# Nikhil-Kulkarni/RayTrace-miniapp

Measured on AMD Instinct MI355X. Metric: ray_steps_per_sec, higher is better.
Workload: dtype f32+f64

## Files before the change

### raytrace-miniapp_amd/csrc/rt_launch.hip

```cpp
#include "rt_path.hip"
#include "rt_freq.hip"
#include "rt_fused.hip"
#include "rt_spec.hip"
#include "rt_step.hip"
#include "rt_step_seeds.hip"
#include "rt_fused_step.hip"
#include "rt_step_scan.hip"
#include "rt_step_scan_seeds.hip"
#include "rt_step_ase_seeds.hip"

#include "rt_runtime.h"
#include "rt_run_shape.h"

#include <atomic>
#include <cstdlib>
#include <cstring>
#include <map>
#include <mutex>

using namespace rtr;

namespace {

int allow_lds(const void *kernel, int device, size_t bytes, size_t limit)
// ... 707 lines not shown
        out->pass_nslot      = s.nslot;
        out->pass_lds        = s.flds;
        out->pass_grid       = s.fgrid;
        out->pass_fetch_shift = s.fetch_shift;
        return RT_OK;
    }
    const PassKind kind   = pass_kind(f);
    const PassShape ps    = pass_shape(kind, f, t);
    out->pass_kind        = (int) kind;
    out->pass_wg_waves    = ps.wg_waves;
    out->pass_in_lds      = ps.in_lds;
    out->pass_nslot       = ps.nslot;
    out->pass_lds         = ps.lds;
    out->pass_grid        = ps.grid;
    out->pass_fetch_shift = ps.fetch_shift;
    return RT_OK;
}

#ifdef RT_WAVETIMES
int rt_hip_debug_wavetimes(unsigned long long *summary8, unsigned long long *end8192, unsigned long long *dry8192)
{
    HIP_TRY(hipDeviceSynchronize());
    HIP_TRY(hipMemcpyFromSymbol(summary8, HIP_SYMBOL(rt::g_wt), 8 * sizeof(unsigned long long)));
    HIP_TRY(hipMemcpyFromSymbol(end8192, HIP_SYMBOL(rt::g_wt_end), 8192 * sizeof(unsigned long long)));
    HIP_TRY(hipMemcpyFromSymbol(dry8192, HIP_SYMBOL(rt::g_wt_dry), 8192 * sizeof(unsigned long long)));
    unsigned long long init[8] = { ~0ull, 0, ~0ull, 0, ~0ull, 0, 0, 0 };
    HIP_TRY(hipMemcpyToSymbol(HIP_SYMBOL(rt::g_wt), init, sizeof(init)));
    return RT_OK;
}
int rt_hip_debug_wavetrace(unsigned long long *trace, int samples, unsigned *blocks)
{
    HIP_TRY(hipDeviceSynchronize());
    if (samples != rt::WT_TRACE)
        return fail_arg("rt_hip_debug_wavetrace: samples");
    if (blocks)
        HIP_TRY(hipMemcpyFromSymbol(blocks, HIP_SYMBOL(rt::g_wt_blocks), sizeof(unsigned) * 8192 * rt::WT_TRACE * 6));
    HIP_TRY(hipMemcpyFromSymbol(trace, HIP_SYMBOL(rt::g_wt_trace), sizeof(unsigned long long) * 8192 * rt::WT_TRACE));
    void *sym = nullptr;
    HIP_TRY(hipGetSymbolAddress(&sym, HIP_SYMBOL(rt::g_wt_trace)));
    HIP_TRY(hipMemset(sym, 0, sizeof(unsigned long long) * 8192 * rt::WT_TRACE));
    return RT_OK;
}
int rt_hip_debug_publish(unsigned long long *pub4, unsigned long long *vm)
{
    HIP_TRY(hipDeviceSynchronize());
    HIP_TRY(hipMemcpyFromSymbol(pub4, HIP_SYMBOL(rt::g_wt_pub), sizeof(unsigned long long) * 8192 * 4));
    HIP_TRY(hipMemcpyFromSymbol(vm, HIP_SYMBOL(rt::g_wt_vm), sizeof(unsigned long long) * 8192));
    void *sym = nullptr;
    HIP_TRY(hipGetSymbolAddress(&sym, HIP_SYMBOL(rt::g_wt_pub)));
    HIP_TRY(hipMemset(sym, 0, sizeof(unsigned long long) * 8192 * 4));
    HIP_TRY(hipGetSymbolAddress(&sym, HIP_SYMBOL(rt::g_wt_vm)));
    HIP_TRY(hipMemset(sym, 0, sizeof(unsigned long long) * 8192));
    return RT_OK;
}
int rt_hip_debug_freqtimes(unsigned long long *times, unsigned *n_waves)
{
    HIP_TRY(hipDeviceSynchronize());
    HIP_TRY(hipMemcpyFromSymbol(times, HIP_SYMBOL(rt::g_ft), 6 * 8192 * sizeof(unsigned long long)));
    HIP_TRY(hipMemcpyFromSymbol(n_waves, HIP_SYMBOL(rt::g_ft_n), sizeof(unsigned)));
    const unsigned zero = 0;
    HIP_TRY(hipMemcpyToSymbol(HIP_SYMBOL(rt::g_ft_n), &zero, sizeof(zero)));
    return RT_OK;
}
#endif

#ifdef RT_INSTRUMENT
int rt_hip_debug_ray_iters(unsigned short *out, unsigned long long n)
{
    HIP_TRY(hipDeviceSynchronize());
    HIP_TRY(hipMemcpyFromSymbol(out, HIP_SYMBOL(rt::g_ray_iters), (size_t) n * sizeof(unsigned short)));
    return RT_OK;
}
#endif
#ifdef RT_INSTRUMENT
int rt_hip_debug_prune_counters(unsigned long long *out4)
{
    HIP_TRY(hipDeviceSynchronize());
    HIP_TRY(hipMemcpyFromSymbol(out4, HIP_SYMBOL(rt::g_prune), 4 * sizeof(unsigned long long)));
    unsigned long long z[4] = { 0 };
    HIP_TRY(hipMemcpyToSymbol(HIP_SYMBOL(rt::g_prune), z, sizeof(z)));
    return RT_OK;
}
#endif
#if defined(RT_INSTRUMENT) || defined(RT_TIMEBLOCKS)
int rt_hip_debug_counters(unsigned long long *out8)
{
    HIP_TRY(hipDeviceSynchronize());
    HIP_TRY(hipMemcpyFromSymbol(out8, HIP_SYMBOL(rt::g_inst), 8 * sizeof(unsigned long long)));
    unsigned long long z[8] = { 0 };
    HIP_TRY(hipMemcpyToSymbol(HIP_SYMBOL(rt::g_inst), z, sizeof(z)));
    return RT_OK;
}
#endif

}
```

### raytrace-miniapp_amd/csrc/rt_march.hip

```cpp
#pragma once
#include "rt_math.h"

#include <cfloat>

namespace rt {

enum : int { ST_IDLE = 0, ST_CELL = 1, ST_XSETUP = 2, ST_STEP = 3, ST_DONE = 4 };

typedef double f64x2 __attribute__((ext_vector_type(2)));
typedef float f32x4 __attribute__((ext_vector_type(4)));
typedef unsigned u32x4 __attribute__((ext_vector_type(4)));

__device__ __forceinline__ unsigned div_magic(unsigned x, unsigned mul, unsigned sh)
{
    return mul ? __umulhi(x, mul) >> sh : x;
}
__device__ __forceinline__ void grid_index(const DevRays &R, unsigned ridx, unsigned &i, unsigned &j, unsigned &k,
                                           unsigned &m)
{
    const unsigned ijkm = (unsigned) (R.first + (long long) ridx * R.stride);
    const unsigned q1   = div_magic(ijkm, R.div_mul[0], R.div_sh[0]);
    m                   = ijkm - q1 * (unsigned) R.ngb;
    const unsigned q2   = div_magic(q1, R.div_mul[1], R.div_sh[1]);
    k                   = q1 - q2 * (unsigned) R.nga;
    i                   = div_magic(q2, R.div_mul[2], R.div_sh[2]);
    j                   = q2 - i * (unsigned) R.ngy;
}

__device__ __forceinline__ void load_ray(const DevRays &R, unsigned ridx, rt_ray &ray, float &ta, float &tb,
                                         bool want_tan)
{
    if (R.list) {
        ray = R.list[ridx];
        if (want_tan) {
            ta = R.sxy[2 * (size_t) ridx];
            tb = R.sxy[2 * (size_t) ridx + 1];
        }
    } else {
        unsigned i, j, k, m;
        grid_index(R, ridx, i, j, k, m);
        ray.x      = (float) R.gx[i];
        ray.y      = (float) R.gy[j];
        ray.a      = (float) R.ga[k];
        ray.b      = (float) R.gb[m];
        if (want_tan) {
            ta = R.tan_a[k];
            tb = R.tan_b[m];
        }
    }
}

__device__ __attribute__((noinline)) float tan_wide(float x)
{
    if (!(fabsf(x) <= FLT_MAX))
        return x - x;
    return (float) tan((double) x);
}
__device__ __attribute__((noinline)) float atan_wide(float x)
{
    const float A0 = 3.3333334327e-01f, A1 = -2.0000000298e-01f, A2 = 1.4285714924e-01f, A3 = -1.1111110449e-01f,
                A4 = 9.0908870101e-02f, A5 = -7.6918758452e-02f, A6 = 6.6610731184e-02f, A7 = -5.8335702866e-02f,
                A8 = 4.9768779427e-02f, A9 = -3.6531571299e-02f, A10 = 1.6285819933e-02f;
    const unsigned hx = __float_as_uint(x), ix = hx & 0x7fffffffu;
    const bool neg = (hx >> 31) != 0u;
    if (ix >= 0x4c000000u) {
        if (ix > 0x7f800000u)
            return x + x;
        const float r = 1.5707962513e+00f + 7.5497894159e-08f;
        return neg ? -r : r;
    }
    float hi, lo;
    x = fabsf(x);
    if (ix < 0x3f980000u) {
        if (ix < 0x3f300000u) {
            hi = 4.6364760399e-01f;
            lo = 5.0121582440e-09f;
            x  = (2.0f * x - 1.0f) / (2.0f + x);
        } else {
            hi = 7.8539812565e-01f;
            lo = 3.7748947079e-08f;
            x  = (x - 1.0f) / (x + 1.0f);
        }
    } else {
        if (ix < 0x401c0000u) {
            hi = 9.8279368877e-01f;
            lo = 3.4473217170e-08f;
            x  = (x - 1.5f) / (1.0f + 1.5f * x);
        } else {
            hi = 1.5707962513e+00f;
            lo = 7.5497894159e-08f;
// ... 165 lines not shown
    const unsigned long long nth = (unsigned long long) gridDim.x * blockDim.x;
    for (unsigned long long t = tid; t < (unsigned long long) n_fast + n_other; t += nth) {
        const unsigned u = t < n_fast ? lo + (unsigned) t : (unsigned) (t - n_fast) << 8;
        float q          = __uint_as_float(u);
        const float a    = inv_norm(q);
        asm volatile("" : "+v"(q));
        const float b = 1.0f / sqrtf(q);
        checked++;
        if (__float_as_uint(a) != __float_as_uint(b) && !(a != a && b != b))
            bad++;
    }
    for (unsigned long long t = tid; t < (4ull << 23); t += nth) {
        float n       = __uint_as_float(0x3e800000u + (unsigned) t);
        const float a = fdiv_one_nr(n);
        asm volatile("" : "+v"(n));
        const float b = 1.0f / n;
        checked++;
        bad += __float_as_uint(a) != __float_as_uint(b) ? 1 : 0;
    }
    for (unsigned long long t = tid; t < (1ull << 28); t += nth) {
        const unsigned h0 = selftest_hash((unsigned) t * 2u + 1u), h1 = selftest_hash((unsigned) t * 2u + 0x9e3779b9u);
        const int ea = -84 + (int) (h0 % 84u), eb = -78 + (int) (h1 % 122u);
        if (ea - eb >= 96 || eb - ea >= 96 || ea - eb < -120)
            continue;
        float x = __uint_as_float(((unsigned) (ea + 127) << 23) | (selftest_hash(h0) & 0x7fffffu));
        float y = __uint_as_float(((unsigned) (eb + 127) << 23) | (selftest_hash(h1) & 0x7fffffu));
        const float a = fdiv_nr(x, y);
        asm volatile("" : "+v"(x), "+v"(y));
        const float b = x / y;
        checked++;
        bad += __float_as_uint(a) != __float_as_uint(b) ? 1 : 0;
    }
    if (tid == 0) {
        float inf = __uint_as_float(0x7f800000u), qnan = __uint_as_float(0x7fc00000u), big = 3.0e38f;
        asm volatile("" : "+v"(inf), "+v"(qnan), "+v"(big));
        const unsigned pio2 = 0x3fc90fdbu;
        const float t0 = tanf_flt32_kernel(inf), t1 = tanf_flt32_kernel(-inf), t2 = tanf_flt32_kernel(qnan), t3 = tan_wide(inf),
                    t4 = tan_wide(qnan), t5 = tanf_flt32_kernel(big);
        const float a0 = atanf_flt32_kernel(inf), a1 = atanf_flt32_kernel(-inf), a2 = atanf_flt32_kernel(qnan),
                    a3 = atanf_flt32_kernel(big), a4 = atanf_flt32_kernel(-big);
        checked += 11;
        bad += (t0 == t0) + (t1 == t1) + (t2 == t2) + (t3 == t3) + (t4 == t4) + (__float_as_uint(t5) == 0x7fc12345u);
        bad += (__float_as_uint(a0) != pio2) + (__float_as_uint(a1) != (pio2 | 0x80000000u)) + (a2 == a2) +
               (__float_as_uint(a3) != pio2) + (__float_as_uint(a4) != (pio2 | 0x80000000u));
    }
    atomicAdd(&counts[0], checked);
    atomicAdd(&counts[1], bad);
}

extern "C" __global__ void __launch_bounds__(256) rt_tan_kernel(const rt_ray *rays, unsigned long long n, float *sxy)
{
    unsigned long long i = (unsigned long long) blockIdx.x * blockDim.x + threadIdx.x;
    if (i < n) {
        rt_ray r       = rays[i];
        sxy[2 * i]     = tanf_flt32_kernel(1e-3f * r.a);
        sxy[2 * i + 1] = tanf_flt32_kernel(1e-3f * r.b);
    }
}

__device__ __forceinline__ int bisect_interval(const Interval *iv, int n, double v)
{
    int lo = 0, hi = n - 1;
    while (hi - lo != 1) {
        int mid = (hi + lo) / 2;
        if (iv[mid].hi >= v)
            hi = mid;
        else
            lo = mid;
    }
    return hi;
}
__device__ __forceinline__ int guess_interval(int n, float g0, float inv_h, float v)
{
    return (int) fminf(fmaxf((v - g0) * inv_h, 0.0f), (float) (n - 2)) + 1;
}

#ifdef RT_INSTRUMENT
__device__ unsigned long long g_inst[8];
__device__ unsigned long long g_prune[4];
__device__ unsigned short g_ray_iters[1u << 23];
#endif
#ifdef RT_TIMEBLOCKS
__device__ unsigned long long g_inst[8];
#endif
#ifdef RT_WAVETIMES
__device__ unsigned long long g_wt[8];
__device__ unsigned long long g_wt_end[8192], g_wt_dry[8192];
constexpr int WT_TRACE = 64;
__device__ unsigned long long g_wt_trace[8192][WT_TRACE];
__device__ unsigned g_wt_blocks[8192][WT_TRACE][6];
__device__ unsigned long long g_wt_pub[8192][4];
__device__ unsigned long long g_wt_vm[8192];
#endif
#if defined(RT_INSTRUMENT) || defined(RT_TIMEBLOCKS) || defined(RT_WAVETIMES)
struct MarchDiag {
    static __device__ __forceinline__ unsigned wave_number() { return blockIdx.x * (blockDim.x >> 6) + (threadIdx.x >> 6); }
    static __device__ __forceinline__ bool first_active_lane()
    {
        return (int) (threadIdx.x & 63) == __ffsll((long long) __ballot(1)) - 1;
    }
#ifdef RT_INSTRUMENT
    unsigned w[3] = { 0, 0, 0 }, a[3] = { 0, 0, 0 }, ray_iters = 0;
#endif
#if defined(RT_TIMEBLOCKS) || defined(RT_WAVEBLOCKS)
    unsigned long long tb_acc[6] = { 0, 0, 0, 0, 0, 0 }, tb_last = __builtin_readcyclecounter(), tb_iters = 0;
#endif
#ifdef RT_WAVETIMES
    const unsigned long long wt_start = __builtin_amdgcn_s_memrealtime();
    unsigned long long wt_dry = 0, pub_t0 = 0;
    unsigned wt_a_runs = 0, wt_b_runs = 0, wave_iter = 0;
#endif
    __device__ __forceinline__ void tick(int i)
    {
#ifdef RT_INSTRUMENT
        a[i]++;
        w[i] += first_active_lane() ? 1u : 0u;
#endif
    }
    __device__ __forceinline__ void mark(int i)
    {
#if defined(RT_TIMEBLOCKS) || defined(RT_WAVEBLOCKS)
        const unsigned long long now = __builtin_readcyclecounter();
        tb_acc[i] += now - tb_last;
        tb_last = now;
#endif
    }
    __device__ __forceinline__ void iteration(int st, int lane, int n_idle)
    {
#ifdef RT_INSTRUMENT
        ray_iters += st != ST_IDLE ? 1u : 0u;
#endif
#ifdef RT_TIMEBLOCKS
        tb_iters++;
#endif
#ifdef RT_WAVETIMES
        if ((++wave_iter & 15u) == 0u) {
            const unsigned wid = wave_number(), smp = wave_iter >> 4;
            if (lane == 0 && wid < 8192u && smp < (unsigned) WT_TRACE) {
                g_wt_trace[wid][smp] = (__builtin_amdgcn_s_memrealtime() & 0xffffffffffull) | ((unsigned long long) (WAVE - n_idle) << 40) |
                                       ((unsigned long long) wt_a_runs << 48) | ((unsigned long long) wt_b_runs << 56);
                g_wt_trace[wid][0] = smp;
#ifdef RT_WAVEBLOCKS
                for (int b = 0; b < 6; b++)
                    g_wt_blocks[wid][smp][b] = (unsigned) tb_acc[b];
#endif
            }
#ifdef RT_WAVEBLOCKS
            for (int b = 0; b < 6; b++)
                tb_acc[b] = 0;
#endif
            wt_a_runs = wt_b_runs = 0;
        }
#endif
    }
    __device__ __forceinline__ void counters_dry()
    {
#ifdef RT_WAVETIMES
        wt_dry = __builtin_amdgcn_s_memrealtime();
#endif
    }
    __device__ __forceinline__ void blocks_run(bool a_runs, bool lane_wants_b)
    {
#ifdef RT_WAVETIMES
        wt_a_runs += a_runs ? 1u : 0u;
        wt_b_runs += __ballot(lane_wants_b) != 0ull ? 1u : 0u;
#endif
    }
    __device__ __forceinline__ void ray_retired(unsigned ridx)
    {
#ifdef RT_INSTRUMENT
        if (ridx < (1u << 23))
            g_ray_iters[ridx] = (unsigned short) (ray_iters < 65535u ? ray_iters : 65535u);
        ray_iters = 0;
#endif
    }
    __device__ __forceinline__ void publish_begin()
    {
#ifdef RT_WAVETIMES
        pub_t0 = __builtin_amdgcn_s_memrealtime();
#endif
    }
    __device__ __forceinline__ void publish_stores_landed()
    {
#ifdef RT_WAVETIMES
        const unsigned long long now = __builtin_amdgcn_s_memrealtime();
        atomicAdd(&g_wt_vm[wave_number() & 8191u], now - pub_t0);
        pub_t0 = now;
#endif
    }
    __device__ __forceinline__ void publish_end()
    {
#ifdef RT_WAVETIMES
        const unsigned long long dt = __builtin_amdgcn_s_memrealtime() - pub_t0;
        unsigned long long *q       = g_wt_pub[wave_number() & 8191u];
        atomicAdd(&q[0], dt);
        atomicAdd(&q[1], 1ull);
        atomicMax(&q[3], dt);
#endif
    }
    static __device__ __forceinline__ void push_retry()
    {
#ifdef RT_WAVETIMES
        atomicAdd(&g_wt_pub[wave_number() & 8191u][2], 1ull);
#endif
    }
    __device__ __forceinline__ void tiny_dividend()
    {
#ifdef RT_INSTRUMENT
        if (first_active_lane())
            atomicAdd(&g_inst[6], 1ull);
#endif
    }
    __device__ __forceinline__ void prune(int i)
    {
#ifdef RT_INSTRUMENT
        if (first_active_lane())
            atomicAdd(&g_prune[i], 1ull);
#endif
    }
    __device__ __forceinline__ void wave_end(int lane)
    {
#ifdef RT_WAVETIMES
        if (lane == 0) {
            const unsigned long long wt_end = __builtin_amdgcn_s_memrealtime();
            atomicMin(&g_wt[0], wt_start);
            atomicMax(&g_wt[1], wt_start);
            const unsigned n = atomicAdd((unsigned *) &g_wt[6], 1u);
            if (n < 8192)
                g_wt_end[n] = wt_end | ((unsigned long long) (threadIdx.x >> 6) << 56), g_wt_dry[n] = wt_dry;
        }
#endif
#ifdef RT_TIMEBLOCKS
        if (lane == 0) {
            for (int i = 0; i < 6; i++)
                atomicAdd(&g_inst[i], tb_acc[i]);
            atomicAdd(&g_inst[7], tb_iters);
        }
#endif
#ifdef RT_INSTRUMENT
        for (int i = 0; i < 3; i++) {
            const unsigned tw = wave_sum_u32(w[i]), ta = wave_sum_u32(a[i]);
            if (lane == 0) {
                atomicAdd(&g_inst[2 * i], (unsigned long long) tw);
                atomicAdd(&g_inst[2 * i + 1], (unsigned long long) ta);
            }
        }
#endif
    }
};
#else
struct MarchDiag {
    __device__ __forceinline__ void tick(int) {}
    __device__ __forceinline__ void mark(int) {}
    __device__ __forceinline__ void iteration(int, int, int) {}
    __device__ __forceinline__ void counters_dry() {}
    __device__ __forceinline__ void blocks_run(bool, bool) {}
    __device__ __forceinline__ void ray_retired(unsigned) {}
    __device__ __forceinline__ void publish_begin() {}
    __device__ __forceinline__ void publish_stores_landed() {}
    __device__ __forceinline__ void publish_end() {}
    static __device__ __forceinline__ void push_retry() {}
    __device__ __forceinline__ void tiny_dividend() {}
    __device__ __forceinline__ void prune(int) {}
    __device__ __forceinline__ void wave_end(int) {}
};
#endif

struct TileList {
    unsigned *head;
    unsigned *next;
    unsigned *lnode;
    unsigned *nalloc;
    unsigned cap;
    unsigned *rem;
    unsigned *marching;
    unsigned n_waves;
    unsigned split;
    unsigned k_part;
};
constexpr unsigned TILE_NONE = 0xffffffffu;
constexpr unsigned TILE_PART_FLAG = 1u << 30, TILE_PART_SHIFT = 28, TILE_ID_MASK = (1u << TILE_PART_SHIFT) - 1u;
__device__ __forceinline__ unsigned tile_node(unsigned entry)
{
    return (entry & TILE_ID_MASK) * 4u + ((entry & TILE_PART_FLAG) ? (entry >> TILE_PART_SHIFT) & 3u : 0u);
}
constexpr unsigned TILE_REF_GLOBAL = 1u << 31;
__device__ __forceinline__ void tile_push(const TileList &T, unsigned tile)
{
    const unsigned id = __hip_atomic_fetch_add(T.nalloc, 1u, __ATOMIC_RELAXED, __HIP_MEMORY_SCOPE_WORKGROUP);
    unsigned old      = __hip_atomic_load(T.head, __ATOMIC_RELAXED, __HIP_MEMORY_SCOPE_WORKGROUP);
    if (id < T.cap) {
        __hip_atomic_store(&T.lnode[2u * id], tile, __ATOMIC_RELAXED, __HIP_MEMORY_SCOPE_WORKGROUP);
        for (;;) {
            __hip_atomic_store(&T.lnode[2u * id + 1u], old, __ATOMIC_RELAXED, __HIP_MEMORY_SCOPE_WORKGROUP);
            asm volatile("s_waitcnt lgkmcnt(0)" ::: "memory");
            if (__hip_atomic_compare_exchange_strong(T.head, &old, id, __ATOMIC_RELAXED, __ATOMIC_RELAXED, __HIP_MEMORY_SCOPE_WORKGROUP))
                return;
            MarchDiag::push_retry();
        }
    }
    tile |= TILE_REF_GLOBAL;
    for (;;) {
        __hip_atomic_store(&T.next[tile_node(tile & ~TILE_REF_GLOBAL)], old, __ATOMIC_RELAXED, __HIP_MEMORY_SCOPE_WORKGROUP);
        asm volatile("s_waitcnt vmcnt(0)" ::: "memory");
        if (__hip_atomic_compare_exchange_strong(T.head, &old, tile, __ATOMIC_RELAXED, __ATOMIC_RELAXED, __HIP_MEMORY_SCOPE_WORKGROUP))
            return;
        MarchDiag::push_retry();
    }
}
__device__ __forceinline__ void tile_publish(const TileList &T, unsigned tile)
{
    bool parts = T.split == 2u;
    if (T.split == 1u)
        parts = __hip_atomic_load(T.head, __ATOMIC_RELAXED, __HIP_MEMORY_SCOPE_WORKGROUP) == TILE_NONE &&
                __hip_atomic_load(T.marching, __ATOMIC_RELAXED, __HIP_MEMORY_SCOPE_WORKGROUP) * 8u <= T.n_waves;
    if (parts && T.k_part != 0u) {
        for (unsigned q = 0; q < 4u; q++)
            tile_push(T, tile | (q << TILE_PART_SHIFT) | TILE_PART_FLAG);
    } else {
        tile_push(T, tile);
    }
}
__device__ __forceinline__ unsigned tile_pop(const TileList &T)
{
    unsigned old = __hip_atomic_load(T.head, __ATOMIC_RELAXED, __HIP_MEMORY_SCOPE_WORKGROUP);
    while (old != TILE_NONE) {
        const unsigned nxt = (old & TILE_REF_GLOBAL)
                                 ? __hip_atomic_load(&T.next[tile_node(old & ~TILE_REF_GLOBAL)], __ATOMIC_RELAXED, __HIP_MEMORY_SCOPE_WORKGROUP)
                                 : __hip_atomic_load(&T.lnode[2u * old + 1u], __ATOMIC_RELAXED, __HIP_MEMORY_SCOPE_WORKGROUP);
        if (__hip_atomic_compare_exchange_strong(T.head, &old, nxt, __ATOMIC_RELAXED, __ATOMIC_RELAXED, __HIP_MEMORY_SCOPE_WORKGROUP))
            break;
    }
    if (old == TILE_NONE)
        return TILE_NONE;
    return (old & TILE_REF_GLOBAL) ? (old & ~TILE_REF_GLOBAL) : __hip_atomic_load(&T.lnode[2u * old], __ATOMIC_RELAXED, __HIP_MEMORY_SCOPE_WORKGROUP);
}

template <bool LDS_TAB> __device__ __forceinline__ void march_load_tables(const DevParams &P, unsigned char *lds_raw)
{
    if (LDS_TAB) {
        const uint4 *src = reinterpret_cast<const uint4 *>(P.blob);
        uint4 *dst       = reinterpret_cast<uint4 *>(lds_raw);
        const unsigned n16 = P.blob_bytes / 16, step = blockDim.x;
        for (unsigned i0 = threadIdx.x; i0 < n16; i0 += 8 * step) {
            uint4 v[8];
#pragma unroll
            for (int u = 0; u < 8; u++) {
                const unsigned i = i0 + (unsigned) u * step;
                v[u]             = src[i < n16 ? i : i0];
            }
#pragma unroll
            for (int u = 0; u < 8; u++) {
                const unsigned i = i0 + (unsigned) u * step;
                if (i < n16)
                    dst[i] = v[u];
            }
        }
        __syncthreads();
    }
}

enum : int { MARCH_OPT_PRUNE = 1, MARCH_OPT_NO_NTEST = 2, MARCH_OPT_PRUNE_H24 = 4, MARCH_OPT_SCAN = 8 };
constexpr unsigned SCAN_BND_BYTES = 20u, SCAN_BND_ROW = WAVE * SCAN_BND_BYTES;
RT_HD inline size_t scan_bnd_off(unsigned ridx, int j, int L)
{
    return ((size_t) (ridx >> 6) * (size_t) (L - 1) + (size_t) (j - 1)) * SCAN_BND_ROW + (size_t) (ridx & 63u) * SCAN_BND_BYTES;
}
RT_HD inline size_t scan_bnd_bytes(unsigned long long n_rays, int L)
{
    return (size_t) ((n_rays + WAVE - 1) / WAVE) * (size_t) (L > 1 ? L - 1 : 0) * SCAN_BND_ROW;
}
template <bool LDS_TAB, bool BOUNDED, bool FUSED, int MODE = 0, int OPT = 0>
__device__ __forceinline__ void march_wave(const DevParams &P, unsigned char *lds_raw, const TileList done)
{
    const int lane        = lane_id();
    const int L           = P.L;
    const int S           = L * RT_N_SUB;
    const unsigned n_rays = P.ray_end;
    const bool backward   = MODE == 1 ? true : ((MODE == 2 || MODE == 3) ? false : P.method == 1);
    const bool use_emis   = MODE == 1 ? true : ((MODE == 2 || MODE == 4) ? false : P.use_emis != 0);
    const bool path_on    = MODE == 0 ? P.path_on != 0 : false;
    const unsigned CH     = P.chunk;
    constexpr int REFILL  = 8;

    const unsigned char *tab = LDS_TAB ? lds_raw : P.blob;
    const BlobGain *hdr = reinterpret_cast<const BlobGain *>(tab);
    const unsigned lds_base = LDS_TAB ? (unsigned) (size_t) (__attribute__((address_space(3))) unsigned char *) lds_raw : 0u;

    static_assert(RT_N_SUB == 3, "sub-segment ends are tabulated for three sub-segments");
    float zs0 = (P.dz0 * (0.0f + 1.0f) / RT_N_SUB), zs1 = (P.dz0 * (1.0f + 1.0f) / RT_N_SUB),
          zs2 = (P.dz0 * (2.0f + 1.0f) / RT_N_SUB);
    asm volatile("" : "+v"(zs0), "+v"(zs1), "+v"(zs2));

    unsigned chunk_next = 0, chunk_end = 0;
    unsigned fetched_end = 0, cur_slot = 0;
    unsigned cslot       = 0;
    bool more           = true;
    const unsigned n_launch_rays = n_rays - P.ray_begin;
    const unsigned n_chunks      = (n_launch_rays + CH - 1) / CH;
    unsigned shard = blockIdx.x & 7u, shards_seen_empty = 0;
    const unsigned n_main = n_chunks - (P.late_chunks < n_chunks ? P.late_chunks : 0u);
    const bool late_wave  = (unsigned) __builtin_amdgcn_readfirstlane((int) (threadIdx.x >> 6)) - P.late_first < P.late_waves;
    unsigned zone = 0;

    int st        = ST_IDLE;
    unsigned ridx = 0;
    int seg = 0, iz = 0, ii = 0;
    float z = 0.0f, z_stop = 0.0f;
    float px = 0, py = 0, pz = 0, sx = 0, sy = 0, sz = 1;
    float gacc = 0, eacc = 0;
    int cell_last = 0, sub = 0;
    unsigned char *recp = P.rec;
    unsigned lane12     = 0;
    BlobGain G    = hdr[1];
    unsigned steps = 0;
    bool escaped = false, mirror = false;
    unsigned any_bits = 0;
    int c00 = 0;
    float f00 = 1, f10 = 1, f01 = 1, f11 = 1;
    double dnx0 = 0, dnx1 = 0, dny0 = 0, dny1 = 0;
    f64x2 ix0 = { 0.0, 1.0 }, iy0 = { 0.0, 1.0 };
    f32x4 ix1 = { 1.0f, 0.0f, 0.0f, 0.0f }, iy1 = { 1.0f, 0.0f, 0.0f, 0.0f };
    float g0 = 0, E0 = 0;
    float dzrem = 0, zc = 0, path = 0;
    float rx = 0, ry = 0, rz = 0, n = 0, n0 = 0, gxn = 0, gyn = 0, lim2 = 0, dzcap = 0, hsum = 0;
    unsigned tot_steps = 0, tot_esc = 0, tot_rays = 0, tot_skip = 0;
    unsigned spin = 0;
    MarchDiag diag;
    for (;;) {
        diag.mark(5);
        unsigned long long idle2      = __ballot(st == ST_IDLE);
        const unsigned long long idle = idle2;
        const int n_idle              = (int) __popcll(idle);
        diag.iteration(st, lane, n_idle);
        if (!BOUNDED) {
            if (((++spin) & 0xfffu) == 0u && spin >= P.spin_limit) {
                spin = 0;
                if (st != ST_IDLE) {
                    escaped = true;
                    sx = sy = sz = 0.0f;
                    st           = ST_CELL;
                }
            }
        }
        if (more && (n_idle >= REFILL)) {
            const int rank = (int) __builtin_amdgcn_mbcnt_hi((unsigned) (idle >> 32),
                                                             __builtin_amdgcn_mbcnt_lo((unsigned) idle, 0u));
            int need = n_idle, off = 0;
            bool got = false;
            while (need > 0) {
                if (chunk_next == chunk_end && !(FUSED && chunk_next != fetched_end)) {
                    unsigned c = 0;
                    if (lane == 0)
                        c = atomicAdd(&P.ctl->next_tile[P.launch_id][shard][zone * 8u], 1u);
                    c = (unsigned) __builtin_amdgcn_readfirstlane((int) c) * 8u + shard + zone * n_main;
                    if (c >= (zone ? n_chunks : n_main)) {
                        if (++shards_seen_empty == 8) {
                            if (zone == 0u && late_wave && n_main < n_chunks) {
                                zone              = 1u;
                                shards_seen_empty = 0;
                                continue;
                            }
                            more = false;
                            diag.counters_dry();
                            break;
                        }
                        shard = (shard + 1) & 7u;
                        continue;
                    }
                    chunk_next = P.ray_begin + c * CH;
                    chunk_end  = (n_rays - chunk_next < CH) ? n_rays : chunk_next + CH;
                    if (FUSED) {
                        fetched_end = chunk_end;
                        chunk_end   = chunk_next;
                    }
                }
                if (FUSED && chunk_next == chunk_end) {
                    const unsigned in_use    = lane < 32 ? __hip_atomic_load(&done.rem[lane], __ATOMIC_RELAXED, __HIP_MEMORY_SCOPE_WAVEFRONT) : 1u;
                    const unsigned slot_busy = ~(unsigned) __ballot(lane < 32 && in_use == 0u);
                    const int fs = __builtin_ffs((int) ~slot_busy) - 1;
                    if (fs < 0)
                        break;
                    chunk_end = fetched_end - chunk_next < (unsigned) WAVE ? fetched_end : chunk_next + (unsigned) WAVE;
                    cur_slot  = (unsigned) fs;
                    if (lane == 0)
                        __hip_atomic_store(&done.rem[fs], chunk_end - chunk_next, __ATOMIC_RELAXED, __HIP_MEMORY_SCOPE_WAVEFRONT);
                }
                int avail = (int) (chunk_end - chunk_next);
                int take  = avail < need ? avail : need;
                if (st == ST_IDLE && !got && rank >= off && rank < off + take) {
                    ridx = chunk_next + (unsigned) (rank - off);
                    got  = true;
                    if (FUSED)
                        cslot = cur_slot;
                }
                chunk_next += (unsigned) take;
                need -= take;
                off += take;
            }
            if (!BOUNDED && __ballot(got) != 0ull)
                spin = 0;
            if (got) {
                rt_ray ray;
                float ta = 0, tb = 0;
                load_ray(P.rays, ridx, ray, ta, tb, true);
                px = ray.x;
                py = ray.y;
                pz = 0.0f;
                sx = ta;
                sy = tb;
                sz = 1.0f;
                if (backward) {
                    sx = -sx;
                    sy = -sy;
                    sz = -sz;
                }
                renormalise(sx, sy, sz);
                const BlobGain G0 = hdr[backward ? P.N - 1 : 1];
                const float dsum  = sx + sy + sz;
                const bool wild   = ((px != px) | (py != py) | (dsum != dsum)) &
                                  !((px < G0.lo_x) | (px > G0.hi_x) | (py < G0.lo_y) | (py > G0.hi_y));
                if (path_on) {
                    float *pp = P.path + (size_t) ridx * 3 * (size_t) (S + 1) + 3 * (size_t) (backward ? S : 0);
                    pp[0]     = px;
                    pp[1]     = py;
                }
                recp      = P.rec + rec_slot_off(ridx, backward ? S - 1 : 0, P.rec_stride);
                lane12    = (ridx & 63u) * 12u;
                seg       = 0;
                iz        = 0;
                ii        = backward ? P.N - 1 : 1;
                G         = G0;
                z         = 0.0f;
                z_stop    = zs0;
                gacc      = 0.0f;
                eacc      = 0.0f;
                cell_last = 0;
                steps     = 0;
                escaped   = wild;
                sx        = wild ? 0.0f : sx;
                sy        = wild ? 0.0f : sy;
                sz        = wild ? 0.0f : sz;
                any_bits  = P.no_skip;
                sub       = 0;
                st        = ST_CELL;
            }
            idle2 = __ballot(st == ST_IDLE);
        }
        if (idle2 == ~0ull) {
            if (!more)
                break;
        } else {

        diag.mark(0);
        const unsigned long long want_a = __ballot(st == ST_CELL);
        int park_at = (int) P.park;
        if (!more || (int) P.park > 12 || REFILL > 8) {
            const int n_live = WAVE - (int) __popcll(idle2);
            const int fifth  = (n_live * 13 + 63) >> 6;
            park_at          = fifth < (int) P.park ? fifth : (int) P.park;
        }
        const bool do_a = (int) __popcll(want_a) >= park_at || (~(idle2 | want_a)) == 0ull;
        diag.blocks_run(do_a && want_a != 0ull, st == ST_XSETUP);
        if (do_a && st == ST_CELL) {
            bool in_seg        = !escaped & (z < 0.995f * z_stop);
            if (!in_seg) {
#ifndef RT_ABL_NOSTORE
                *reinterpret_cast<RecSlot *>(recp) = RecSlot{ gacc, eacc, cell_last };
#endif
                recp += backward ? -(int) REC_SLOT_ROW : (int) REC_SLOT_ROW;
                any_bits |= (__float_as_uint(gacc) | __float_as_uint(eacc)) & 0x7fffffffu;
                if (path_on) {
                    float *pp = P.path + (size_t) ridx * 3 * (size_t) (S + 1);
                    for (int zz = iz; zz < (escaped ? RT_N_SUB : iz + 1); zz++) {
                        const int idx = RT_N_SUB * (ii - 1) + (backward ? RT_N_SUB - zz - 1 : zz + 1);
                        pp[3 * idx]     = px;
                        pp[3 * idx + 1] = py;
                    }
                }
                gacc      = 0.0f;
                eacc      = 0.0f;
                cell_last = 0;
                sub++;
                const bool wrap = iz == RT_N_SUB - 1;
                const bool fin  = escaped | (sub == S);
                iz              = wrap ? 0 : iz + 1;
                z               = wrap ? 0.0f : z;
                st              = fin ? ST_DONE : ST_CELL;
                if (wrap & !fin) {
                    if (OPT & MARCH_OPT_SCAN) {
                        unsigned char *bnd = reinterpret_cast<unsigned char *>(((unsigned long long) P.pad_march[1] << 32) | (unsigned long long) P.pad_march[0]);
                        float *q           = reinterpret_cast<float *>(bnd + scan_bnd_off(ridx, seg + 1, L));
                        q[0]               = px;
                        q[1]               = py;
                        q[2]               = sx;
                        q[3]               = sy;
                        q[4]               = sz;
                    }
                    seg++;
                    ii = backward ? P.N - seg - 1 : seg + 1;
                    G  = hdr[ii];
                }
                z_stop = iz == 0 ? zs0 : (iz == 1 ? zs1 : zs2);
                in_seg = !fin & (z < 0.995f * z_stop);
            }
            diag.mark(1);
            if ((st == ST_CELL) & in_seg) {
                if ((px < G.lo_x) | (px > G.hi_x) | (py < G.lo_y) | (py > G.hi_y) | (sz * sz <= 0.01f)) {
                    escaped = true;
                } else {
                    mirror              = G.mirror_y != 0;
                    const Interval *ivx = reinterpret_cast<const Interval *>(tab + G.off_ix);
                    const Interval *ivy = reinterpret_cast<const Interval *>(tab + G.off_iy);
                    f64x2 tx, ty;
                    u32x4 q00, q10, q01, q11;
                    auto gather = [&](int k1, int k2, int c) {
                        const unsigned ox = (unsigned) G.off_ix + (unsigned) k1 * (unsigned) sizeof(Interval);
                        const unsigned oy = (unsigned) G.off_iy + (unsigned) k2 * (unsigned) sizeof(Interval);
                        const unsigned oa = (unsigned) G.off_node + (unsigned) c * (unsigned) sizeof(Node);
                        const unsigned ob = oa + (unsigned) G.Nx * (unsigned) sizeof(Node);
                        if (LDS_TAB) {
                            asm volatile("ds_read_b128 %0, %10\n\t"
                                         "ds_read_b128 %1, %10 offset:16\n\t"
                                         "ds_read_b128 %2, %10 offset:32\n\t"
                                         "ds_read_b128 %3, %11\n\t"
                                         "ds_read_b128 %4, %11 offset:16\n\t"
                                         "ds_read_b128 %5, %11 offset:32\n\t"
                                         "ds_read_b128 %6, %12\n\t"
                                         "ds_read_b128 %7, %12 offset:16\n\t"
                                         "ds_read_b128 %8, %13\n\t"
                                         "ds_read_b128 %9, %13 offset:16\n\t"
                                         "s_waitcnt lgkmcnt(0)"
                                         : "=&v"(ix0), "=&v"(ix1), "=&v"(tx), "=&v"(iy0), "=&v"(iy1), "=&v"(ty), "=&v"(q00), "=&v"(q10),
                                           "=&v"(q01), "=&v"(q11)
                                         : "v"(lds_base + ox), "v"(lds_base + oy), "v"(lds_base + oa), "v"(lds_base + ob));
                        } else {
                            const unsigned char *t = tab;
                            ix0 = *reinterpret_cast<const f64x2 *>(t + ox);
                            ix1 = *reinterpret_cast<const f32x4 *>(t + ox + 16);
                            tx  = *reinterpret_cast<const f64x2 *>(t + ox + 32);
                            iy0 = *reinterpret_cast<const f64x2 *>(t + oy);
                            iy1 = *reinterpret_cast<const f32x4 *>(t + oy + 16);
                            ty  = *reinterpret_cast<const f64x2 *>(t + oy + 32);
                            q00 = *reinterpret_cast<const u32x4 *>(t + oa);
                            q10 = *reinterpret_cast<const u32x4 *>(t + oa + 16);
                            q01 = *reinterpret_cast<const u32x4 *>(t + ob);
                            q11 = *reinterpret_cast<const u32x4 *>(t + ob + 16);
                        }
                    };
                    auto node_n = [](const u32x4 &q) { return __hiloint2double((int) q.y, (int) q.x); };
                    const float ya      = mirror ? fabsf(py) : py;
                    const double pxd = (double) px, yad = (double) ya;
                    int k1     = guess_interval(G.Nx, G.x0f, G.inv_hxf, px);
                    int k2     = guess_interval(G.Ny, G.y0f, G.inv_hyf, ya);
                    c00        = (k1 - 1) + (k2 - 1) * G.Nx;
                    gather(k1, k2, c00);
                    const bool ok = ((k1 == 1) | (ix0.x < pxd)) & ((k1 == G.Nx - 1) | (tx.x >= pxd)) &
                                    ((k2 == 1) | (iy0.x < yad)) & ((k2 == G.Ny - 1) | (ty.x >= yad));
                    if (!ok) {
                        k1  = bisect_interval(ivx, G.Nx, pxd);
                        k2  = bisect_interval(ivy, G.Ny, yad);
                        c00 = (k1 - 1) + (k2 - 1) * G.Nx;
                        gather(k1, k2, c00);
                    }
                    const double n00 = node_n(q00), n10 = node_n(q10), n01 = node_n(q01), n11 = node_n(q11);
                    f00       = (float) n00;
                    f10       = (float) n10;
                    f01       = (float) n01;
                    f11       = (float) n11;
                    dnx0      = n10 - n00;
                    dnx1      = n11 - n01;
                    dny0      = n01 - n00;
                    dny1      = n11 - n10;
                    const float u = (float) div_by_recip<true>(pxd - ix0.x, tx.x - ix0.x, tx.y);
                    const float v = (float) div_by_recip<true>(yad - iy0.x, ty.x - iy0.x, ty.y);
                    g0            = lerp2(u, v, __uint_as_float(q00.z), __uint_as_float(q10.z), __uint_as_float(q01.z),
                                          __uint_as_float(q11.z));
                    E0            = 0.0f;
                    if (use_emis) {
                        E0 = lerp2(u, v, __uint_as_float(q00.w), __uint_as_float(q10.w), __uint_as_float(q01.w),
                                   __uint_as_float(q11.w));
                        E0 = E0 >= 0 ? E0 : 0.0f;
                    }
                    pz    = 0.0f;
                    zc    = 0.0f;
                    path  = 0.0f;
                    dzrem = z_stop - z;
                    if ((px > ix1.y) & (px < ix1.z) & (ya > iy1.y) & (ya < iy1.z) & (dzrem > 0.0f)) {
                        st = ST_XSETUP;
                    } else {
                        z += fabsf(pz);
                        gacc += g0 * path;
                        eacc += E0 * path;
                        cell_last = c00;
                        steps++;
                        diag.tick(2);
                    }
                }
            }
            diag.mark(2);
            if (st == ST_DONE) {
                unsigned fl = F_VALID;
                if (escaped)
                    fl |= F_ESCAPED;
                if (use_emis && any_bits == 0u)
                    fl |= F_SKIP;
                RecMeta m;
                m.px          = px;
                m.py          = py;
                m.sx          = sx;
                m.sy          = sy;
                m.sz          = sz;
                m.flags_steps = fl | ((unsigned) sub << REC_NDONE_SHIFT) |
                                ((steps < 0xfffffu ? steps : 0xfffffu) << REC_STEPS_SHIFT);
                unsigned char *metap = recp + (int) REC_SLOT_ROW * (backward ? sub + 1 : S - sub) + lane12;
#ifndef RT_ABL_NOMETA
                *reinterpret_cast<RecMeta *>(metap) = m;
#else
                if (m.px == 1234.5f)
                    *reinterpret_cast<RecMeta *>(metap) = m;
#endif
                diag.ray_retired(ridx);
                tot_steps += steps;
                tot_esc += escaped ? 1u : 0u;
                tot_skip += (fl & F_SKIP) ? 1u : 0u;
                tot_rays++;
                st = ST_IDLE;
                if (FUSED) {
                    if (__hip_atomic_fetch_add(&done.rem[cslot], 0xffffffffu, __ATOMIC_RELAXED, __HIP_MEMORY_SCOPE_WAVEFRONT) == 1u) {
                        diag.publish_begin();
                        asm volatile("s_waitcnt vmcnt(0)" ::: "memory");
                        diag.publish_stores_landed();
                        tile_publish(done, ridx >> 6);
                        diag.publish_end();
                    }
                }
            }
        }
        diag.mark(3);
        if (st == ST_XSETUP) {
            const float ya   = mirror ? fabsf(py) : py;
            const double dwx = (double) ix1.x, dwy = (double) iy1.x;
            const double xc0 = ix0.x, yc0 = iy0.x, rwx = ix0.y, rwy = iy0.y;
            const float u    = (float) div_by_recip<true>((double) px - xc0, dwx, rwx);
            const float v    = (float) div_by_recip<true>((double) ya - yc0, dwy, rwy);
            n0  = lerp2(u, v, f00, f10, f01, f11);
            gxn = (float) (div_by_recip<true>((1.0 - (double) v) * dnx0, dwx, rwx) +
                           div_by_recip<true>((double) v * dnx1, dwx, rwx));
            gyn = (float) (div_by_recip<true>((1.0 - (double) u) * dny0, dwy, rwy) +
                           div_by_recip<true>((double) u * dny1, dwy, rwy));
            if (mirror && py < 0)
                gyn = -gyn;
            lim2  = dzrem - zc;
            dzcap = P.c_cap * lim2;
            rx    = 0.0f;
            ry    = 0.0f;
            rz    = 0.0f;
            n     = n0;
            hsum  = 0.0f;
            st    = ST_STEP;
            diag.tick(1);
        }

        diag.mark(4);
        if (st == ST_STEP) {
            const float lim0 = 0.1f * ix1.x, lim1 = 0.1f * iy1.x;
            bool run;
            {
                n        = n0 + rx * gxn + ry * gyn;
#ifdef RT_ABL_FASTDIV
#define RT_FDIV(a, b) ((a) * __builtin_amdgcn_rcpf(b))
#else
#define RT_FDIV(a, b) ((a) / (b))
#endif
                const float rn = BOUNDED ? fdiv_one_nr(n) : RT_FDIV(1.0f, n);
                float a0 = sx * gxn + sy * gyn + 1e-12f;
                float t  = BOUNDED ? fmaf(fmaf(-n, a0 * rn, a0), rn, a0 * rn) : div_by_recip_signed(a0, n, rn);
                float qx = div_by_recip_signed(gxn, n, rn);
                float qy = div_by_recip_signed(gyn, n, rn);
#ifndef RT_ABL_NOGUARD
                if (__ballot(fminf(fminf(fabsf(a0), fabsf(gxn)), fabsf(gyn)) < 1e-29f) != 0ull) {
                    diag.tiny_dividend();
                    if (fabsf(a0) < 1e-29f && a0 != 0.0f) {
                        asm volatile("" : "+v"(a0));
                        t = a0 / n;
                    }
                    if (fabsf(gxn) < 1e-29f && gxn != 0.0f) {
                        float g = gxn;
                        asm volatile("" : "+v"(g));
                        qx = g / n;
                    }
                    if (fabsf(gyn) < 1e-29f && gyn != 0.0f) {
                        float g = gyn;
                        asm volatile("" : "+v"(g));
                        qy = g / n;
                    }
                }
#endif
                float fx = qx - sx * t;
                float fy = qy - sy * t;
                float fz = -sz * t;
                float h;
                if (BOUNDED && (OPT & MARCH_OPT_PRUNE)) {
                    const float kd = 1.00002f * dzcap;
                    const float at = fabsf(t), az = fabsf(sz);
                    const float n2 = 1.0001f * (lim2 - fabsf(rz));
                    const float n4 = P.c_h3 * (fabsf(sy) + 5e-4f), d4 = fabsf(fy) + 1e-8f;
                    h = fmin_nan_drop(fdiv_nr(P.c_h3 * (fabsf(sx) + 5e-4f), (fabsf(fx) + 1e-8f)), dzcap);
                    diag.prune(3);
                    if (__ballot(!(P.c_h1 > kd * at)) != 0ull) {
                        h = fmin_nan_drop(fdiv_nr(P.c_h1, at), h);
                        diag.prune(0);
                    }
                    if (!(OPT & MARCH_OPT_PRUNE_H24) || __ballot(!(n2 > kd * az) | !(n4 > kd * d4)) != 0ull) {
                        h = fmin_nan_drop(fmin_nan_drop(fdiv_nr(n2, az), fdiv_nr(n4, d4)), h);
                        diag.prune(1);
                    }
                } else if (BOUNDED) {
                    const float h1 = fdiv_nr(P.c_h1, fabsf(t));
                    const float h2 = fdiv_nr(1.0001f * (lim2 - fabsf(rz)), fabsf(sz));
                    const float h3 = fdiv_nr(P.c_h3 * (fabsf(sx) + 5e-4f), (fabsf(fx) + 1e-8f));
                    const float h4 = fdiv_nr(P.c_h3 * (fabsf(sy) + 5e-4f), (fabsf(fy) + 1e-8f));
// ... 73 lines not shown
```

Baseline: 29.94 billion.

## Defer ray retirement into the refill block to batch record writes

```diff
diff --git a/raytrace-miniapp_amd/csrc/rt_launch.hip b/raytrace-miniapp_amd/csrc/rt_launch.hip
--- a/raytrace-miniapp_amd/csrc/rt_launch.hip
+++ b/raytrace-miniapp_amd/csrc/rt_launch.hip
@@ -813,6 +813,16 @@
     return RT_OK;
 }
 #endif
+#ifdef RT_TIMEBLOCKS
+int rt_hip_debug_retire_counters(unsigned long long *out4)
+{
+    HIP_TRY(hipDeviceSynchronize());
+    HIP_TRY(hipMemcpyFromSymbol(out4, HIP_SYMBOL(rt::g_retire), 4 * sizeof(unsigned long long)));
+    unsigned long long z[4] = { 0 };
+    HIP_TRY(hipMemcpyToSymbol(HIP_SYMBOL(rt::g_retire), z, sizeof(z)));
+    return RT_OK;
+}
+#endif
 #if defined(RT_INSTRUMENT) || defined(RT_TIMEBLOCKS)
 int rt_hip_debug_counters(unsigned long long *out8)
 {
diff --git a/raytrace-miniapp_amd/csrc/rt_march.hip b/raytrace-miniapp_amd/csrc/rt_march.hip
--- a/raytrace-miniapp_amd/csrc/rt_march.hip
+++ b/raytrace-miniapp_amd/csrc/rt_march.hip
@@ -5,7 +5,7 @@
 
 namespace rt {
 
-enum : int { ST_IDLE = 0, ST_CELL = 1, ST_XSETUP = 2, ST_STEP = 3, ST_DONE = 4 };
+enum : int { ST_DONE = -1, ST_IDLE = 0, ST_CELL = 1, ST_XSETUP = 2, ST_STEP = 3 };
 
 typedef double f64x2 __attribute__((ext_vector_type(2)));
 typedef float f32x4 __attribute__((ext_vector_type(4)));
@@ -337,6 +337,7 @@
 #endif
 #ifdef RT_TIMEBLOCKS
 __device__ unsigned long long g_inst[8];
+__device__ unsigned long long g_retire[4];
 #endif
 #ifdef RT_WAVETIMES
 __device__ unsigned long long g_wt[8];
@@ -360,6 +361,9 @@
 #if defined(RT_TIMEBLOCKS) || defined(RT_WAVEBLOCKS)
     unsigned long long tb_acc[6] = { 0, 0, 0, 0, 0, 0 }, tb_last = __builtin_readcyclecounter(), tb_iters = 0;
 #endif
+#ifdef RT_TIMEBLOCKS
+    unsigned rt_fin = 0, rt_blk = 0, rt_refill = 0, rt_dry = 0;
+#endif
 #ifdef RT_WAVETIMES
     const unsigned long long wt_start = __builtin_amdgcn_s_memrealtime();
     unsigned long long wt_dry = 0, pub_t0 = 0;
@@ -383,7 +387,7 @@
     __device__ __forceinline__ void iteration(int st, int lane, int n_idle)
     {
 #ifdef RT_INSTRUMENT
-        ray_iters += st != ST_IDLE ? 1u : 0u;
+        ray_iters += st > ST_IDLE ? 1u : 0u;
 #endif
 #ifdef RT_TIMEBLOCKS
         tb_iters++;
@@ -421,6 +425,25 @@
         wt_b_runs += __ballot(lane_wants_b) != 0ull ? 1u : 0u;
 #endif
     }
+    __device__ __forceinline__ void finishing(int st)
+    {
+#ifdef RT_TIMEBLOCKS
+        rt_fin += (__ballot(st == ST_DONE) != 0ull && first_active_lane()) ? 1u : 0u;
+#endif
+    }
+    __device__ __forceinline__ void retire_block(int st, bool more)
+    {
+#ifdef RT_TIMEBLOCKS
+        rt_blk += __ballot(st == ST_DONE) != 0ull ? 1u : 0u;
+        rt_dry += more ? 0u : 1u;
+#endif
+    }
+    __device__ __forceinline__ void refill()
+    {
+#ifdef RT_TIMEBLOCKS
+        rt_refill++;
+#endif
+    }
     __device__ __forceinline__ void ray_retired(unsigned ridx)
     {
 #ifdef RT_INSTRUMENT
@@ -486,10 +509,15 @@
         }
 #endif
 #ifdef RT_TIMEBLOCKS
+        const unsigned fin_wave = wave_sum_u32(rt_fin);
         if (lane == 0) {
             for (int i = 0; i < 6; i++)
                 atomicAdd(&g_inst[i], tb_acc[i]);
             atomicAdd(&g_inst[7], tb_iters);
+            atomicAdd(&g_retire[0], (unsigned long long) fin_wave);
+            atomicAdd(&g_retire[1], (unsigned long long) rt_blk);
+            atomicAdd(&g_retire[2], (unsigned long long) rt_refill);
+            atomicAdd(&g_retire[3], (unsigned long long) rt_dry);
         }
 #endif
 #ifdef RT_INSTRUMENT
@@ -510,6 +538,9 @@
     __device__ __forceinline__ void iteration(int, int, int) {}
     __device__ __forceinline__ void counters_dry() {}
     __device__ __forceinline__ void blocks_run(bool, bool) {}
+    __device__ __forceinline__ void finishing(int) {}
+    __device__ __forceinline__ void retire_block(int, bool) {}
+    __device__ __forceinline__ void refill() {}
     __device__ __forceinline__ void ray_retired(unsigned) {}
     __device__ __forceinline__ void publish_begin() {}
     __device__ __forceinline__ void publish_stores_landed() {}
@@ -651,6 +682,7 @@
     unsigned fetched_end = 0, cur_slot = 0;
     unsigned cslot       = 0;
     bool more           = true;
+    unsigned refill_at = (unsigned) REFILL;
     const unsigned n_launch_rays = n_rays - P.ray_begin;
     const unsigned n_chunks      = (n_launch_rays + CH - 1) / CH;
     unsigned shard = blockIdx.x & 7u, shards_seen_empty = 0;
@@ -684,123 +716,168 @@
     MarchDiag diag;
     for (;;) {
         diag.mark(5);
-        unsigned long long idle2      = __ballot(st == ST_IDLE);
+        unsigned long long idle2      = __ballot(st <= ST_IDLE);
         const unsigned long long idle = idle2;
-        const int n_idle              = (int) __popcll(idle);
+        int n_idle                    = (int) __popcll(idle);
+        asm volatile("" : "+s"(n_idle));
         diag.iteration(st, lane, n_idle);
         if (!BOUNDED) {
             if (((++spin) & 0xfffu) == 0u && spin >= P.spin_limit) {
                 spin = 0;
-                if (st != ST_IDLE) {
+                if (st > ST_IDLE) {
                     escaped = true;
                     sx = sy = sz = 0.0f;
                     st           = ST_CELL;
                 }
             }
         }
-        if (more && (n_idle >= REFILL)) {
-            const int rank = (int) __builtin_amdgcn_mbcnt_hi((unsigned) (idle >> 32),
-                                                             __builtin_amdgcn_mbcnt_lo((unsigned) idle, 0u));
-            int need = n_idle, off = 0;
-            bool got = false;
-            while (need > 0) {
-                if (chunk_next == chunk_end && !(FUSED && chunk_next != fetched_end)) {
-                    unsigned c = 0;
-                    if (lane == 0)
-                        c = atomicAdd(&P.ctl->next_tile[P.launch_id][shard][zone * 8u], 1u);
-                    c = (unsigned) __builtin_amdgcn_readfirstlane((int) c) * 8u + shard + zone * n_main;
-                    if (c >= (zone ? n_chunks : n_main)) {
-                        if (++shards_seen_empty == 8) {
-                            if (zone == 0u && late_wave && n_main < n_chunks) {
-                                zone              = 1u;
-                                shards_seen_empty = 0;
-                                continue;
+        if ((unsigned) n_idle >= refill_at) {
+            diag.mark(0);
+            diag.retire_block(st, more);
+            if (st == ST_DONE) {
+                unsigned fl = F_VALID;
+                if (escaped)
+                    fl |= F_ESCAPED;
+                if (use_emis && any_bits == 0u)
+                    fl |= F_SKIP;
+                RecMeta m;
+                m.px          = px;
+                m.py          = py;
+                m.sx          = sx;
+                m.sy          = sy;
+                m.sz          = sz;
+                m.flags_steps = fl | ((unsigned) sub << REC_NDONE_SHIFT) |
+                                ((steps < 0xfffffu ? steps : 0xfffffu) << REC_STEPS_SHIFT);
+                unsigned char *metap = recp + (int) REC_SLOT_ROW * (backward ? sub + 1 : S - sub) + lane12;
+#ifndef RT_ABL_NOMETA
+                *reinterpret_cast<RecMeta *>(metap) = m;
+#else
+                if (m.px == 1234.5f)
+                    *reinterpret_cast<RecMeta *>(metap) = m;
+#endif
+                diag.ray_retired(ridx);
+                tot_steps += steps;
+                tot_esc += escaped ? 1u : 0u;
+                tot_skip += (fl & F_SKIP) ? 1u : 0u;
+                tot_rays++;
+                st = ST_IDLE;
+                if (FUSED) {
+                    if (__hip_atomic_fetch_add(&done.rem[cslot], 0xffffffffu, __ATOMIC_RELAXED, __HIP_MEMORY_SCOPE_WAVEFRONT) == 1u) {
+                        diag.publish_begin();
+                        asm volatile("s_waitcnt vmcnt(0)" ::: "memory");
+                        diag.publish_stores_landed();
+                        tile_publish(done, ridx >> 6);
+                        diag.publish_end();
+                    }
+                }
+            }
+            diag.mark(3);
+            if (more) {
+                diag.refill();
+                const int rank = (int) __builtin_amdgcn_mbcnt_hi((unsigned) (idle >> 32),
+                                                                 __builtin_amdgcn_mbcnt_lo((unsigned) idle, 0u));
+                int need = n_idle, off = 0;
+                bool got = false;
+                while (need > 0) {
+                    if (chunk_next == chunk_end && !(FUSED && chunk_next != fetched_end)) {
+                        unsigned c = 0;
+                        if (lane == 0)
+                            c = atomicAdd(&P.ctl->next_tile[P.launch_id][shard][zone * 8u], 1u);
+                        c = (unsigned) __builtin_amdgcn_readfirstlane((int) c) * 8u + shard + zone * n_main;
+                        if (c >= (zone ? n_chunks : n_main)) {
+                            if (++shards_seen_empty == 8) {
+                                if (zone == 0u && late_wave && n_main < n_chunks) {
+                                    zone              = 1u;
+                                    shards_seen_empty = 0;
+                                    continue;
+                                }
+                                more = false;
+                                refill_at = 0u;
+                                diag.counters_dry();
+                                break;
                             }
-                            more = false;
-                            diag.counters_dry();
+                            shard = (shard + 1) & 7u;
+                            continue;
+                        }
+                        chunk_next = P.ray_begin + c * CH;
+                        chunk_end  = (n_rays - chunk_next < CH) ? n_rays : chunk_next + CH;
+                        if (FUSED) {
+                            fetched_end = chunk_end;
+                            chunk_end   = chunk_next;
+                        }
+                    }
+                    if (FUSED && chunk_next == chunk_end) {
+                        const unsigned in_use    = lane < 32 ? __hip_atomic_load(&done.rem[lane], __ATOMIC_RELAXED, __HIP_MEMORY_SCOPE_WAVEFRONT) : 1u;
+                        const unsigned slot_busy = ~(unsigned) __ballot(lane < 32 && in_use == 0u);
+                        const int fs = __builtin_ffs((int) ~slot_busy) - 1;
+                        if (fs < 0)
                             break;
-                        }
-                        shard = (shard + 1) & 7u;
-                        continue;
-                    }
-                    chunk_next = P.ray_begin + c * CH;
-                    chunk_end  = (n_rays - chunk_next < CH) ? n_rays : chunk_next + CH;
-                    if (FUSED) {
-                        fetched_end = chunk_end;
-                        chunk_end   = chunk_next;
-                    }
+                        chunk_end = fetched_end - chunk_next < (unsigned) WAVE ? fetched_end : chunk_next + (unsigned) WAVE;
+                        cur_slot  = (unsigned) fs;
+                        if (lane == 0)
+                            __hip_atomic_store(&done.rem[fs], chunk_end - chunk_next, __ATOMIC_RELAXED, __HIP_MEMORY_SCOPE_WAVEFRONT);
+                    }
+                    int avail = (int) (chunk_end - chunk_next);
+                    int take  = avail < need ? avail : need;
+                    if (st == ST_IDLE && !got && rank >= off && rank < off + take) {
+                        ridx = chunk_next + (unsigned) (rank - off);
+                        got  = true;
+                        if (FUSED)
+                            cslot = cur_slot;
+                    }
+                    chunk_next += (unsigned) take;
+                    need -= take;
+                    off += take;
                 }
-                if (FUSED && chunk_next == chunk_end) {
-                    const unsigned in_use    = lane < 32 ? __hip_atomic_load(&done.rem[lane], __ATOMIC_RELAXED, __HIP_MEMORY_SCOPE_WAVEFRONT) : 1u;
-                    const unsigned slot_busy = ~(unsigned) __ballot(lane < 32 && in_use == 0u);
-                    const int fs = __builtin_ffs((int) ~slot_busy) - 1;
-                    if (fs < 0)
-                        break;
-                    chunk_end = fetched_end - chunk_next < (unsigned) WAVE ? fetched_end : chunk_next + (unsigned) WAVE;
-                    cur_slot  = (unsigned) fs;
-                    if (lane == 0)
-                        __hip_atomic_store(&done.rem[fs], chunk_end - chunk_next, __ATOMIC_RELAXED, __HIP_MEMORY_SCOPE_WAVEFRONT);
+                if (!BOUNDED && __ballot(got) != 0ull)
+                    spin = 0;
+                if (got) {
+                    rt_ray ray;
+                    float ta = 0, tb = 0;
+                    load_ray(P.rays, ridx, ray, ta, tb, true);
+                    px = ray.x;
+                    py = ray.y;
+                    pz = 0.0f;
+                    sx = ta;
+                    sy = tb;
+                    sz = 1.0f;
+                    if (backward) {
+                        sx = -sx;
+                        sy = -sy;
+                        sz = -sz;
+                    }
+                    renormalise(sx, sy, sz);
+                    const BlobGain G0 = hdr[backward ? P.N - 1 : 1];
+                    const float dsum  = sx + sy + sz;
+                    const bool wild   = ((px != px) | (py != py) | (dsum != dsum)) &
+                                      !((px < G0.lo_x) | (px > G0.hi_x) | (py < G0.lo_y) | (py > G0.hi_y));
+                    if (path_on) {
+                        float *pp = P.path + (size_t) ridx * 3 * (size_t) (S + 1) + 3 * (size_t) (backward ? S : 0);
+                        pp[0]     = px;
+                        pp[1]     = py;
+                    }
+                    recp      = P.rec + rec_slot_off(ridx, backward ? S - 1 : 0, P.rec_stride);
+                    lane12    = (ridx & 63u) * 12u;
+                    seg       = 0;
+                    iz        = 0;
+                    ii        = backward ? P.N - 1 : 1;
+                    G         = G0;
+                    z         = 0.0f;
+                    z_stop    = zs0;
+                    gacc      = 0.0f;
+                    eacc      = 0.0f;
+                    cell_last = 0;
+                    steps     = 0;
+                    escaped   = wild;
+                    sx        = wild ? 0.0f : sx;
+                    sy        = wild ? 0.0f : sy;
+                    sz        = wild ? 0.0f : sz;
+                    any_bits  = P.no_skip;
+                    sub       = 0;
+                    st        = ST_CELL;
                 }
-                int avail = (int) (chunk_end - chunk_next);
-                int take  = avail < need ? avail : need;
-                if (st == ST_IDLE && !got && rank >= off && rank < off + take) {
-                    ridx = chunk_next + (unsigned) (rank - off);
-                    got  = true;
-                    if (FUSED)
-                        cslot = cur_slot;
-                }
-                chunk_next += (unsigned) take;
-                need -= take;
-                off += take;
+                idle2 = __ballot(st == ST_IDLE);
             }
-            if (!BOUNDED && __ballot(got) != 0ull)
-                spin = 0;
-            if (got) {
-                rt_ray ray;
-                float ta = 0, tb = 0;
-                load_ray(P.rays, ridx, ray, ta, tb, true);
-                px = ray.x;
-                py = ray.y;
-                pz = 0.0f;
-                sx = ta;
-                sy = tb;
-                sz = 1.0f;
-                if (backward) {
-                    sx = -sx;
-                    sy = -sy;
-                    sz = -sz;
-                }
-                renormalise(sx, sy, sz);
-                const BlobGain G0 = hdr[backward ? P.N - 1 : 1];
-                const float dsum  = sx + sy + sz;
-                const bool wild   = ((px != px) | (py != py) | (dsum != dsum)) &
-                                  !((px < G0.lo_x) | (px > G0.hi_x) | (py < G0.lo_y) | (py > G0.hi_y));
-                if (path_on) {
-                    float *pp = P.path + (size_t) ridx * 3 * (size_t) (S + 1) + 3 * (size_t) (backward ? S : 0);
-                    pp[0]     = px;
-                    pp[1]     = py;
-                }
-                recp      = P.rec + rec_slot_off(ridx, backward ? S - 1 : 0, P.rec_stride);
-                lane12    = (ridx & 63u) * 12u;
-                seg       = 0;
-                iz        = 0;
-                ii        = backward ? P.N - 1 : 1;
-                G         = G0;
-                z         = 0.0f;
-                z_stop    = zs0;
-                gacc      = 0.0f;
-                eacc      = 0.0f;
-                cell_last = 0;
-                steps     = 0;
-                escaped   = wild;
-                sx        = wild ? 0.0f : sx;
-                sy        = wild ? 0.0f : sy;
-                sz        = wild ? 0.0f : sz;
-                any_bits  = P.no_skip;
-                sub       = 0;
-                st        = ST_CELL;
-            }
-            idle2 = __ballot(st == ST_IDLE);
         }
         if (idle2 == ~0ull) {
             if (!more)
@@ -842,6 +919,7 @@
                 iz              = wrap ? 0 : iz + 1;
                 z               = wrap ? 0.0f : z;
                 st              = fin ? ST_DONE : ST_CELL;
+                diag.finishing(st);
                 if (wrap & !fin) {
                     if (OPT & MARCH_OPT_SCAN) {
                         unsigned char *bnd = reinterpret_cast<unsigned char *>(((unsigned long long) P.pad_march[1] << 32) | (unsigned long long) P.pad_march[0]);
@@ -953,46 +1031,8 @@
                     }
                 }
             }
-            diag.mark(2);
-            if (st == ST_DONE) {
-                unsigned fl = F_VALID;
-                if (escaped)
-                    fl |= F_ESCAPED;
-                if (use_emis && any_bits == 0u)
-                    fl |= F_SKIP;
-                RecMeta m;
-                m.px          = px;
-                m.py          = py;
-                m.sx          = sx;
-                m.sy          = sy;
-                m.sz          = sz;
-                m.flags_steps = fl | ((unsigned) sub << REC_NDONE_SHIFT) |
-                                ((steps < 0xfffffu ? steps : 0xfffffu) << REC_STEPS_SHIFT);
-                unsigned char *metap = recp + (int) REC_SLOT_ROW * (backward ? sub + 1 : S - sub) + lane12;
-#ifndef RT_ABL_NOMETA
-                *reinterpret_cast<RecMeta *>(metap) = m;
-#else
-                if (m.px == 1234.5f)
-                    *reinterpret_cast<RecMeta *>(metap) = m;
-#endif
-                diag.ray_retired(ridx);
-                tot_steps += steps;
-                tot_esc += escaped ? 1u : 0u;
-                tot_skip += (fl & F_SKIP) ? 1u : 0u;
-                tot_rays++;
-                st = ST_IDLE;
-                if (FUSED) {
-                    if (__hip_atomic_fetch_add(&done.rem[cslot], 0xffffffffu, __ATOMIC_RELAXED, __HIP_MEMORY_SCOPE_WAVEFRONT) == 1u) {
-                        diag.publish_begin();
-                        asm volatile("s_waitcnt vmcnt(0)" ::: "memory");
-                        diag.publish_stores_landed();
-                        tile_publish(done, ridx >> 6);
-                        diag.publish_end();
-                    }
-                }
-            }
-        }
-        diag.mark(3);
+        }
+        diag.mark(2);
         if (st == ST_XSETUP) {
             const float ya   = mirror ? fabsf(py) : py;
             const double dwx = (double) ix1.x, dwy = (double) iy1.x;
```

Result: faster. 30.47 billion (median of 6 runs) (+1.7%).
